# alberthild/vainplex-openclaw

Measured on NVIDIA B200. Metric: messages_scanned_per_s, higher is better.
Workload: dtype u8

## Files before the change

vainplex_openclaw_b200/csrc/bitprog.h:

```cpp
#pragma once
#include <cstdint>
#include "kernels.h"
#include "pike_vm.h"

namespace cg {

constexpr uint32_t kBitProgNone = 0xffffffffu;
constexpr uint32_t kBitCtxs = 32;
CG_HD uint32_t bitprog_meta_off(uint32_t W) { return (128u + kBitCtxs) * W; }
CG_HD uint32_t bitprog_rows_off(uint32_t W) { return bitprog_meta_off(W) + 7u + 2u * W; }
CG_HD uint32_t bitprog_words(uint32_t W, uint32_t n_rows) { return bitprog_rows_off(W) + n_rows * 64u * W * W; }

CG_HD uint32_t bitprog_ctx(int prev, int next, bool at_start) {
  return (uint32_t)(is_word(prev) != is_word(next)) | (at_start ? 2u : 0u) | (next < 0 ? 4u : 0u);
}
CG_HD uint32_t bitprog_in128(uint64_t lo, uint64_t hi, int u) { return u < 0 || u >= 0x80 ? 0u : (uint32_t)(((u & 64) ? hi : lo) >> (u & 63)) & 1u; }

template <int W>
CG_HD int bitprog_test_w(const uint64_t* __restrict__ bp, const uint8_t* __restrict__ m, uint32_t len, uint32_t s, uint32_t t0, uint32_t max_steps, const uint64_t* __restrict__ resume = nullptr) {
  const uint64_t* accept = bp; const uint64_t* start = bp + 128 * W; const uint64_t* hd = bp + bitprog_meta_off(W); const uint64_t* rows = bp + bitprog_rows_off(W);
  const uint64_t meta = hd[0], map0 = hd[1], map1 = hd[2];
  const bool start_same = (meta >> 8) & 1u, has_look = (meta >> 9) & 1u, one_row = (meta & 15u) == 1u;
  const uint64_t lb0 = has_look ? hd[3] : 0, lb1 = has_look ? hd[4] : 0, la0 = has_look ? hd[5] : 0, la1 = has_look ? hd[6] : 0;
  uint64_t m_next[W], m_self[W], live[W], acc_cur[W], start0[W];
  constexpr uint64_t kMatch = 1ull << 63;
  for (int w = 0; w < W; w++) { m_next[w] = hd[7 + w]; m_self[w] = hd[7 + W + w]; }
  int prev = s > 0 ? (m[s - 1] < 0x80 ? (int)m[s - 1] : 0x80) : -1;
  int cur = s < len ? (int)m[s] : -1;
  uint32_t ctx = bitprog_ctx(prev, cur, s == 0) | (has_look ? bitprog_in128(lb0, lb1, prev) << 3 | bitprog_in128(la0, la1, cur) << 4 : 0u);
  for (int w = 0; w < W; w++) { start0[w] = resume ? 0 : start[ctx * W + w]; live[w] = resume ? resume[w] : start0[w]; acc_cur[w] = cur >= 0 && cur < 0x80 ? accept[cur * W + w] : 0; }
  if (resume) t0 = s - 1;
  for (uint32_t pos = s;;) {
    int nb[4]; uint64_t na[4][W];
#ifdef __CUDA_ARCH__
#pragma unroll
#endif
    for (int i = 0; i < 4; i++) nb[i] = pos + 1 + i < len ? (int)m[pos + 1 + i] : -1;
#ifdef __CUDA_ARCH__
#pragma unroll
#endif
    for (int i = 0; i < 4; i++) for (int w = 0; w < W; w++) na[i][w] = nb[i] >= 0 && nb[i] < 0x80 ? accept[nb[i] * W + w] : 0;
#ifdef __CUDA_ARCH__
#pragma unroll
#endif
    for (int i = 0; i < 4; i++) {
      if (live[W - 1] & kMatch) return 1;
      if (cur < 0) return 0;
      if (cur >= 0x80 || pos - s >= max_steps) return -1;
      const int nxt = nb[i];
      uint64_t hit[W], carry = 0, any_hit = 0;
      for (int w = 0; w < W; w++) {
        const uint64_t h = live[w] & acc_cur[w], hn = h & m_next[w];
        live[w] = (hn << 1) | carry | (h & m_self[w]);
        carry = hn >> 63;
        hit[w] = h & ~(m_next[w] | m_self[w]); any_hit |= hit[w];
      }
      if (!start_same || any_hit) ctx = bitprog_ctx(cur, nxt < 0x80 ? nxt : 0x80, false) | (has_look ? bitprog_in128(lb0, lb1, cur) << 3 | bitprog_in128(la0, la1, nxt) << 4 : 0u);
      if (any_hit) {
        const uint32_t row = one_row ? 0u : (uint32_t)(((ctx & 16u) ? map1 : map0) >> (4 * (ctx & 15u))) & 15u;
        const uint64_t* fw = rows + (size_t)row * 64 * W * W;
        for (int w = 0; w < W; w++) {
          uint64_t hw = hit[w];
          while (hw) {
#if defined(__CUDA_ARCH__)
            const int k = __ffsll((long long)hw) - 1;
#else
            const int k = __builtin_ctzll(hw);
#endif
            hw &= hw - 1;
            for (int v = 0; v < W; v++) live[v] |= fw[(size_t)(w * 64 + k) * W + v];
          }
        }
      }
      pos++;
      if (pos <= t0) { for (int w = 0; w < W; w++) live[w] |= start_same ? start0[w] : start[ctx * W + w]; }
      else { uint64_t any = 0; for (int w = 0; w < W; w++) any |= live[w]; if (!any) return 0; }
      cur = nxt;
      for (int w = 0; w < W; w++) acc_cur[w] = na[i][w];
    }
  }
}
CG_HD int bitprog_test(const uint64_t* __restrict__ bp, const uint8_t* __restrict__ m, uint32_t len, uint32_t s, uint32_t t0, uint32_t max_steps = 0xffffffffu, const uint64_t* __restrict__ resume = nullptr) {
  return bp[0] == 2 ? bitprog_test_w<2>(bp + 1, m, len, s, t0, max_steps, resume) : bitprog_test_w<1>(bp + 1, m, len, s, t0, max_steps, resume);
}

CG_HD uint32_t bitprog_sel8(const uint32_t a[8], uint32_t i) {
  const uint32_t lo = (i & 2u) ? ((i & 1u) ? a[3] : a[2]) : ((i & 1u) ? a[1] : a[0]);
  const uint32_t hi = (i & 2u) ? ((i & 1u) ? a[7] : a[6]) : ((i & 1u) ? a[5] : a[4]);
  return (i & 4u) ? hi : lo;
}

CG_HD uint32_t island_start(const DevRuleset& rs, uint32_t rule, const uint8_t* __restrict__ m, uint32_t len, uint32_t t0, uint32_t pre_units, uint32_t limit = 0xffffffffu) {
  const uint32_t pa = pre_units >> 16; pre_units &= 0xffffu;
  const uint32_t* alpha = pa != 0xffffu ? rs.bytesets + (size_t)pa * 8 : rs.rule_alpha + (size_t)rule * 8;
  if (t0 > len) t0 = len;
  uint32_t s = t0;
  uint32_t floor_ = pre_units < 0xffffu ? (t0 > 3u * pre_units ? t0 - 3u * pre_units : 0u) : 0u;
  if (limit != 0xffffffffu && t0 - floor_ > limit) floor_ = t0 - limit - (t0 > limit ? 1u : 0u);
  if (s <= floor_) return s;
  uint32_t a[8];
#ifdef __CUDA_ARCH__
#pragma unroll
#endif
  for (int i = 0; i < 8; i++) a[i] = alpha[i];
  for (;;) {
    uint32_t b[4];
#ifdef __CUDA_ARCH__
#pragma unroll
#endif
    for (uint32_t i = 0; i < 4; i++) b[i] = s > floor_ + i ? m[s - 1 - i] : 0x100u;
#ifdef __CUDA_ARCH__
#pragma unroll
#endif
    for (uint32_t i = 0; i < 4; i++) {
      if (b[i] > 0xffu || !((bitprog_sel8(a, b[i] >> 5) >> (b[i] & 31u)) & 1u)) return s;
      s--;
    }
  }
}


CG_HD int island_test(const DevRuleset& rs, uint32_t f, uint32_t r, const uint8_t* __restrict__ m, uint32_t len, uint32_t t0, uint32_t pre, uint32_t max_steps) {
  const uint64_t* bp = reinterpret_cast<const uint64_t*>(rs.bit_words) + rs.bit_off[r];
  const uint64_t* resume = nullptr; uint32_t s = 0;
  if (f != 0xffffffffu && rs.factor_skip) {
    const uint64_t* sk = reinterpret_cast<const uint64_t*>(rs.factor_skip) + (size_t)f * 3;
    const uint32_t L = (uint32_t)sk[0];
    if (L && t0 + L <= len) { resume = sk + 1; s = t0 + L; }
  }
  if (!resume) {
    s = island_start(rs, r, m, len, t0, pre, max_steps);
    if (max_steps != 0xffffffffu && (t0 < len ? t0 : len) - s >= max_steps) return -1;
  }
  return bitprog_test(bp, m, len, s, t0, max_steps, resume);
}

}
```

vainplex_openclaw_b200/csrc/capi.cu:

```cuda
#include <cuda_runtime.h>

#include <algorithm>
#include <cstdio>
#include <cstdlib>
#include <cstring>
#include <memory>
#include <dlfcn.h>
#include <mutex>
#include <string>
#include <vector>

#include "../../include/openclaw_gov.h"
#include "kernels.h"
#include "rulec.h"
#include "ruleset_image.h"

using namespace cg;

namespace {

thread_local std::string g_err;
std::mutex g_mu;

struct Ctx {
// ... 58 lines not shown
  std::vector<void*> allocs;
  uint32_t n_sets = 0, program_words = 0;
  ScanWork work{};
  uint64_t seq = 0;
  static constexpr int kMirror = 16;
  uint32_t* h_counters = nullptr; cudaEvent_t e_cnt[kMirror] = {}; bool cnt_pending[kMirror] = {};
  uint32_t grow_l1 = 0, grow_slot = 0, grow_ev = 0;
  uint32_t sticky_flags = 0;
  int verify_ctas = 1;
  void size_verify_grid() { const uint32_t ev = last_counters[1]; if (ev > 2048u) verify_ctas = 4; else if (ev < 256u) verify_ctas = 1; }
  uint32_t last_counters[kCounterWords] = {};
  struct CachedGraph { int kernels = 0; cudaGraphExec_t exec = nullptr; const void* bytes = nullptr; const void* off = nullptr; void* words = nullptr; uint32_t n = 0; uint64_t caps[4] = {0, 0, 0, 0}; uint64_t used = 0; };
  struct OnePath { cudaGraphExec_t exec = nullptr; uint8_t* h_pin = nullptr; uint8_t* d_buf = nullptr; uint64_t caps[4] = {0, 0, 0, 0}; int kernels = 0; } one;
  CachedGraph graphs[2];
  uint64_t graph_clock = 0;
  ~cg_ruleset() {
    for (auto& g : graphs) if (g.exec) cudaGraphExecDestroy(g.exec);
    if (one.exec) cudaGraphExecDestroy(one.exec);
    if (one.h_pin) cudaFreeHost(one.h_pin);
    cudaFree(one.d_buf);
    if (h_counters) cudaFreeHost(h_counters);
    for (auto& e : e_cnt) if (e) cudaEventDestroy(e);
    for (void* p : allocs) cudaFree(p);
    cudaFree(work.heavy_idx); cudaFree(work.l1_pos); cudaFree(work.l1_fac); cudaFree(work.fq); cudaFree(work.slot_of_msg);
    cudaFree(work.counters); cudaFree(work.persist); cudaFree(work.slot_msg); cudaFree(work.cand); cudaFree(work.hit); cudaFree(work.events); cudaFree(work.event_pos); cudaFree(work.event_pre); cudaFree(work.spans);
  }
};

namespace {

template <typename T>
int upload(cg_ruleset* rs, const std::vector<T>& v, const T** out, size_t pad_elems = 4) {
  void* d = nullptr;
  size_t bytes = (v.size() + pad_elems) * sizeof(T);
  CU(cudaMalloc(&d, bytes));
  rs->allocs.push_back(d);
  CU(cudaMemset(d, 0, bytes));
  if (!v.empty()) CU(cudaMemcpy(d, v.data(), v.size() * sizeof(T), cudaMemcpyHostToDevice));
  *out = reinterpret_cast<const T*>(d);
  return CG_OK;
}

int ensure_work(cg_ruleset* rs, ScanWork& w, uint32_t n_msgs, uint32_t l1_cap, uint32_t slot_cap, uint32_t event_cap, uint32_t span_cap) {
  if (!w.counters) { CU(cudaMalloc((void**)&w.counters, kCounterWords * sizeof(uint32_t))); CU(cudaMalloc((void**)&w.persist, 16)); CU(cudaMemset(w.persist, 0, 16)); CU(cudaDeviceSynchronize()); }
  if (n_msgs > w.msg_cap) { cudaFree(w.slot_of_msg); w.slot_of_msg = nullptr; w.msg_cap = 0; CU(cudaMalloc((void**)&w.slot_of_msg, (size_t)n_msgs * 4)); w.msg_cap = n_msgs; }
  if (l1_cap > w.l1_cap) {
    cudaFree(w.l1_pos); cudaFree(w.l1_fac); cudaFree(w.fq); w.l1_pos = w.l1_fac = nullptr; w.fq = nullptr; w.l1_cap = 0;
    CU(cudaMalloc((void**)&w.l1_pos, (size_t)l1_cap * 4)); CU(cudaMalloc((void**)&w.l1_fac, (size_t)l1_cap * 4)); CU(cudaMalloc((void**)&w.fq, (size_t)l1_cap * 8));
    w.l1_cap = l1_cap;
  }
  if (slot_cap > w.slot_cap) {
    cudaFree(w.slot_msg); cudaFree(w.cand); cudaFree(w.hit); w.slot_msg = w.cand = w.hit = nullptr; w.slot_cap = 0;
    size_t rw = rs->dev.rw ? rs->dev.rw : 1;
    CU(cudaMalloc((void**)&w.slot_msg, (size_t)slot_cap * 4));
    CU(cudaMalloc((void**)&w.cand, (size_t)slot_cap * rw * 4));
    CU(cudaMalloc((void**)&w.hit, (size_t)slot_cap * rw * 4));
    CU(cudaMemset(w.cand, 0, (size_t)slot_cap * rw * 4)); CU(cudaMemset(w.hit, 0, (size_t)slot_cap * rw * 4)); CU(cudaMemset(w.persist, 0, 16)); CU(cudaDeviceSynchronize());
    w.slot_cap = slot_cap;
  }
  if (event_cap > w.event_cap) { cudaFree(w.events); cudaFree(w.event_pos); cudaFree(w.event_pre); cudaFree(w.heavy_idx); w.events = nullptr; w.event_pos = w.event_pre = w.heavy_idx = nullptr; w.event_cap = 0; CU(cudaMalloc((void**)&w.events, (size_t)event_cap * sizeof(uint2))); CU(cudaMalloc((void**)&w.heavy_idx, (size_t)event_cap * 4)); CU(cudaMalloc((void**)&w.event_pos, (size_t)event_cap * 4)); CU(cudaMalloc((void**)&w.event_pre, (size_t)event_cap * 4)); w.event_cap = event_cap; }
  if (span_cap > w.span_cap) { cudaFree(w.spans); w.spans = nullptr; w.span_cap = 0; CU(cudaMalloc((void**)&w.spans, (size_t)span_cap * 24)); w.span_cap = span_cap; }
  return CG_OK;
}

static uint32_t scan_pieces() { static const uint32_t k = [] { const char* e = getenv("CG_PIECES"); const int v = e ? atoi(e) : 1; return (uint32_t)(v >= 1 && v <= 4 ? v : 1); }(); return k; }
int run_scan_device(cg_ruleset* rs, const uint8_t* d_bytes, const uint32_t* d_off, uint32_t n, uint64_t* d_words, bool spans, cudaStream_t st) {
  const ScanWork& w = rs->work;
  int k = launch_reset(rs->dev, w, n, G.sm_count, st);
  if (G.profiling) cudaEventRecord(G.pev[0], st);
  const uint32_t K = scan_pieces();
  if (G.profiling) G.prof_pieces = K;
// ... 1212 lines not shown
```

vainplex_openclaw_b200/csrc/kernels.h:

```cpp
#pragma once
#include <cuda_runtime.h>
#include <cstdint>

namespace cg {

struct DevRuleset {
  const uint8_t* image;
  uint32_t image_bytes;
  uint32_t stride;
  uint32_t bm_mask, bloom2;
  uint32_t rk_off, rk_mask;
  uint32_t tables_resident;
  uint32_t dir_off, ent_off;
  uint32_t nb_shift;
  uint32_t n_shapes, shapes[16];
  uint32_t n_trig, trig_byte[2];
  uint32_t hot_c5f, hot_c10, hot_one;
  const uint32_t* trig_offsets;
  const uint32_t* trig_list;
  const uint32_t* bucket_start;
  const uint2* entries;
  const uint4* slots;
  const uint32_t* group_entries;
  uint32_t slot_shift, slot_mask;
// ... 2 lines not shown
  uint32_t max_prog_len;
  uint32_t debug_flags;
  const uint32_t* factors;
  const uint32_t* bytesets;
  const uint32_t* always_rules;
  uint32_t n_always;
  const uint32_t* prog;
  const uint32_t* rule_prog_off;
  const uint32_t* sets;
  const uint16_t* set_ranges;
  const unsigned long long* bit_words; const uint32_t* bit_off;
  const unsigned long long* factor_skip;
  const uint32_t* rule_first;
  const uint32_t* rule_alpha;
  const uint32_t* rule_policy; const uint32_t* rule_action;
  uint32_t n_rules;
  uint32_t rw;
};

struct ScanWork {
  uint32_t* counters;
  uint32_t* l1_pos;
  uint32_t* l1_fac;
  uint2* fq;
  uint32_t* persist;
  uint32_t* slot_of_msg;
  uint32_t* slot_msg;
  uint32_t* cand;
  uint32_t* hit;
  uint2* events;
  uint32_t* heavy_idx;
  uint32_t* event_pos;
  uint32_t* event_pre;
  uint32_t* spans;
  uint32_t l1_cap, msg_cap, slot_cap, event_cap, span_cap;
  uint32_t q_cap, q_slot;
};

enum : uint32_t { ERR_EVENT_OVERFLOW = 1, ERR_SPAN_OVERFLOW = 2, ERR_VM_STACK = 4, ERR_VM_LIST = 8, ERR_SLOT_OVERFLOW = 16, ERR_L1_OVERFLOW = 32 };
constexpr uint32_t kCounterWords = 32;
constexpr uint32_t kConfirmTableBudget = 176u * 1024u;
constexpr uint64_t kWordIncomplete = ~0ull;

int launch_scan(const DevRuleset& rs, const ScanWork& w, const uint8_t* d_bytes, const uint32_t* d_off, uint32_t n,
                uint64_t* d_words, int sm_count, cudaStream_t stream);
int launch_confirm(const DevRuleset& rs, const ScanWork& w, const uint8_t* d_bytes, const uint32_t* d_off, uint32_t n, int sm_count, cudaStream_t stream);
int launch_resolve(const DevRuleset& rs, const ScanWork& w, const uint8_t* d_bytes, const uint32_t* d_off, uint32_t n, bool want_spans, int sm_count, cudaStream_t stream);
int launch_verify(const DevRuleset& rs, const ScanWork& w, const uint8_t* d_bytes, const uint32_t* d_off,
                  bool want_spans, int sm_count, cudaStream_t stream, int ctas_per_sm = 4);
int launch_verdicts(const DevRuleset& rs, const ScanWork& w, uint32_t* d_verdicts, int sm_count, cudaStream_t stream);
int launch_finalize(const DevRuleset& rs, const ScanWork& w, uint64_t* d_words, uint32_t n, int sm_count, cudaStream_t stream);
int launch_reset(const DevRuleset& rs, const ScanWork& w, uint32_t n, int sm_count, cudaStream_t stream);

int launch_pack_one(const DevRuleset& rs, const ScanWork& w, const uint64_t* d_word, uint32_t* d_out, uint32_t rw_cap, cudaStream_t stream);

void prepare_scan_kernels();

int launch_sha256_batch(const uint8_t* d_bytes, const uint64_t* d_off, uint32_t n, uint8_t* d_out, cudaStream_t stream);
int launch_merkle_chain(const uint32_t* d_left, uint32_t n_left, const uint32_t* d_acc_in, uint32_t* d_acc_out, cudaStream_t stream);
int launch_merkle_verify(const uint32_t* d_leaf32, uint64_t index, uint64_t size, const uint32_t* d_path, uint32_t path_len, const uint32_t* d_root32, uint32_t* d_ok, cudaStream_t stream);
int launch_redact_digests(const uint8_t* d_bytes, const uint32_t* d_start, const uint32_t* d_len, uint32_t ns, uint32_t* d_out, cudaStream_t stream);
int launch_redact_splice(const uint8_t* d_bytes, const uint32_t* d_off, const uint32_t* d_out_off, const uint32_t* d_span_begin,
                         const uint32_t* d_span_start, const uint32_t* d_span_len, const uint32_t* d_span_cat, const uint32_t* d_digests,
// ... 11 lines not shown
```

vainplex_openclaw_b200/csrc/scan_kernels.cu:

```cuda
#include "kernels.h"
#include "rulec.h"
#include "pike_vm.h"
#include "bitprog.h"
#include "gram_filter.h"
#include <algorithm>

namespace cg {

__device__ __forceinline__ uint32_t smem_u32(const void* p) { return (uint32_t)__cvta_generic_to_shared(p); }
__device__ __forceinline__ void mbar_init(uint64_t* bar, uint32_t count) {
  asm volatile("mbarrier.init.shared::cta.b64 [%0], %1;" ::"r"(smem_u32(bar)), "r"(count));
}
__device__ __forceinline__ void fence_barrier_init() { asm volatile("fence.mbarrier_init.release.cluster;" ::: "memory"); }
__device__ __forceinline__ void fence_proxy_async() { asm volatile("fence.proxy.async.shared::cta;" ::: "memory"); }
__device__ __forceinline__ void mbar_expect_tx(uint64_t* bar, uint32_t bytes) {
  asm volatile("mbarrier.arrive.expect_tx.shared::cta.b64 _, [%0], %1;" ::"r"(smem_u32(bar)), "r"(bytes) : "memory");
}
__device__ __forceinline__ void tma_bulk_g2s(void* dst, const void* src, uint32_t bytes, uint64_t* bar) {
  asm volatile("cp.async.bulk.shared::cluster.global.mbarrier::complete_tx::bytes [%0], [%1], %2, [%3];"
               ::"r"(smem_u32(dst)), "l"(src), "r"(bytes), "r"(smem_u32(bar)) : "memory");
}
__device__ __forceinline__ void mbar_wait(uint64_t* bar, uint32_t phase) {
  asm volatile(
      "{\n"
// ... 179 lines not shown
    h1 += k;
  };
#pragma unroll 1
  while (c - lane < end_chunk) {
    scan_tile(bA, tA, bB, tB, c);
    scan_tile(bB, tB, bA, tA, c + cstep);
    scan_tile(bA, tA, bB, tB, c + 2u * cstep);
    scan_tile(bB, tB, bA, tA, c + 3u * cstep);
    c += 4u * cstep;
    const uint32_t m = __ballot_sync(FULL, acc != 0);
    if (m) {
      if (acc) asm volatile("st.shared.v2.u32 [%0], {%1, %2};" ::"r"(ring1 + (((t1 + __popc(m & lt)) & (kRing - 1)) << 3)), "r"(c), "r"(acc) : "memory");
      t1 += __popc(m); acc = 0;
      if (t1 - h1 >= 32u) { __syncwarp(); append32(32u); }
    }
  }
  __syncwarp();
  if (t1 != h1) append32(t1 - h1);
}

constexpr uint32_t kIslandSteps = 96;
struct SlotSink {
  const DevRuleset& rs; const ScanWork& w; uint32_t msg; uint32_t slot;
  const uint8_t* text = nullptr; uint32_t text_len = 0;
  __device__ SlotSink(const DevRuleset& r, const ScanWork& wk, uint32_t m, bool ws) : rs(r), w(wk), msg(m), slot(0xffffffffu), want_spans(ws) {}
  __device__ bool ensure_slot() {
    if (slot != 0xffffffffu) return slot < w.slot_cap;
    uint32_t s = *reinterpret_cast<volatile uint32_t*>(&w.slot_of_msg[msg]);
    if (s == 0xffffffffu) {
      uint32_t mine = atomicAdd(&w.counters[0], 1u);
      if (mine >= w.slot_cap) { atomicOr(&w.counters[3], ERR_SLOT_OVERFLOW); slot = mine; return false; }
      w.slot_msg[mine] = msg;
      uint32_t old = atomicCAS(&w.slot_of_msg[msg], 0xffffffffu, mine);
      if (old == 0xffffffffu) s = mine; else { s = old; w.slot_msg[mine] = 0xffffffffu; }
    }
    slot = s;
    return true;
  }
  bool want_spans;
  __device__ void candidate(uint32_t r, uint32_t t0, uint32_t pre, uint32_t f) {
    if (!want_spans && text && rs.bit_words) {
      const uint32_t bo = rs.bit_off[r];
      if (bo != kBitProgNone) {
        if (slot == 0xffffffffu) { const uint32_t s0 = *reinterpret_cast<volatile uint32_t*>(&w.slot_of_msg[msg]); if (s0 != 0xffffffffu && s0 < w.slot_cap && ((w.hit[(size_t)s0 * rs.rw + (r >> 5)] >> (r & 31)) & 1u)) return; }
        const int res = island_test(rs, f, r, text, text_len, t0, pre, kIslandSteps);
        if (res == 0) return;
        if (res == 1) { direct(r); return; }
      }
    }
    if (!ensure_slot()) return;
    uint32_t bit = 1u << (r & 31);
    uint32_t old = atomicOr(&w.cand[(size_t)slot * rs.rw + (r >> 5)], bit);
    if (want_spans && (old & bit)) return;
    uint32_t e = atomicAdd(&w.counters[1], 1u);
    if (e < w.event_cap) {
      const bool heavy = !want_spans && (pre & 0xffffu) >= 24u;
      w.events[e] = make_uint2(slot, r | (heavy ? 0x80000000u : 0u)); w.event_pos[e] = t0; w.event_pre[e] = pre;
      if (heavy) w.heavy_idx[atomicAdd(&w.counters[17], 1u)] = e;
    } else atomicOr(&w.counters[3], ERR_EVENT_OVERFLOW);
  }
  __device__ void candidate_always(uint32_t r) {
    if (!ensure_slot()) return;
    uint32_t bit = 1u << (r & 31);
    uint32_t old = atomicOr(&w.cand[(size_t)slot * rs.rw + (r >> 5)], bit);
    if (old & bit) return;
    uint32_t e = atomicAdd(&w.counters[1], 1u);
    if (e < w.event_cap) { w.events[e] = make_uint2(slot, r); w.event_pos[e] = 0xffffffffu; } else atomicOr(&w.counters[3], ERR_EVENT_OVERFLOW);
  }
  __device__ void direct(uint32_t r) {
    if (!ensure_slot()) return;
    uint32_t bit = 1u << (r & 31);
    atomicOr(&w.cand[(size_t)slot * rs.rw + (r >> 5)], bit);
// ... 128 lines not shown
  uint32_t head = 0, tail = 0, flagged = 0;
  for (uint32_t base = gwarp * 32u; base < nq; base += nwarps * 32u) {
    uint2 q = make_uint2(0u, 0u);
    if (base + lane < nq) q = w.fq[base + lane];
    uint32_t bits = q.y;
    for (;;) {
      const uint32_t m = __ballot_sync(FULL, bits != 0);
      if (!m) break;
      if (bits) {
        const uint32_t bit = (uint32_t)__ffs((int)bits) - 1u; bits &= bits - 1u;
        ring[(tail + __popc(m & lt)) & (kCfRing - 1)] = ((q.x - (bit / kbits + 1u) * cstep) * kbits + (kbits - 1u - bit % kbits)) << kshift;
      }
      tail += __popc(m); flagged += lane == 0 ? __popc(m) : 0u;
      __syncwarp();
      if (tail - head >= 32u) { const uint32_t pos = ring[(head + lane) & (kCfRing - 1)]; head += 32u; __syncwarp(); confirm_gram(c, pos, true); }
    }
  }
  if (tail != head) { const bool a = lane < tail - head; const uint32_t pos = a ? ring[(head + lane) & (kCfRing - 1)] : 0u; __syncwarp(); confirm_gram(c, pos, a); }
  if (c.ptail != c.phead) { const bool a = lane < c.ptail - c.phead; const uint2 pr = a ? c.pring[(c.phead + lane) & (kCfRing - 1)] : make_uint2(0u, 0u); confirm_pairs(c, pr, a); }
  const uint32_t passed = __reduce_add_sync(FULL, c.passed);
  if (lane == 0) { if (flagged) atomicAdd(&w.counters[6], flagged); if (passed) atomicAdd(&w.counters[19], passed); if (c.ptail) atomicAdd(&w.counters[28 + w.q_slot], c.ptail); }
}

__global__ void __launch_bounds__(256, 4)
resolve_kernel(DevRuleset rs, ScanWork w, const uint8_t* __restrict__ bytes, const uint32_t* __restrict__ off, uint32_t n, int want_spans, uint32_t spread) {
  const uint32_t n1 = min(w.counters[4], w.l1_cap);
  const uint32_t stride = gridDim.x * blockDim.x, tid = blockIdx.x * blockDim.x + threadIdx.x;
  for (uint32_t i = tid / spread; i < n1 && tid % spread == 0; i += stride / spread) {
    const uint32_t pos = w.l1_pos[i], f = w.l1_fac[i];
    const uint32_t msg = message_of(off, n, pos);
    if (pos + (rs.factors[(size_t)f * 12 + 1] & 0xffu) > off[msg + 1]) continue;
    SlotSink sink(rs, w, msg, want_spans != 0);
    sink.text = bytes + off[msg]; sink.text_len = off[msg + 1] - off[msg];
    factor_confirmed(rs, f, pos - off[msg], want_spans != 0, sink);
  }
  if (rs.n_always) for (uint32_t msg = tid; msg < n; msg += stride) {
    SlotSink sink(rs, w, msg, want_spans != 0);
    for (uint32_t k = 0; k < rs.n_always; k++) sink.candidate_always(rs.always_rules[k]);
  }
}

constexpr int kVerifyThreads = 64;
constexpr int kVerifyBlock = 256, kVerifyCtasPerSm = 4, kVerifySlots = kVerifyBlock / 32;
constexpr int kSmallProg = 192;

struct GlobalSpanSink {
  const ScanWork& w; uint32_t msg, rule; bool lane0_only;
  __device__ void span(uint32_t sb, uint32_t eb, uint32_t s16, uint32_t e16) {
    if (lane0_only && (threadIdx.x & 31u)) return;
    uint32_t k = atomicAdd(&w.counters[2], 1u);
    if (k < w.span_cap) { uint32_t* o = w.spans + (size_t)k * 6; o[0] = msg; o[1] = rule; o[2] = sb; o[3] = eb; o[4] = s16; o[5] = e16; }
    else atomicOr(&w.counters[3], ERR_SPAN_OVERFLOW);
  }
};

struct SmemStore {
  static constexpr uint32_t cap = kSmallProg;
  static constexpr bool coop = true;
  uint16_t* mark_; uint16_t* pcs_; uint32_t* sts_; uint16_t* stk_; uint32_t stride, t;
  __device__ __forceinline__ uint16_t& mark(uint32_t i) { return mark_[i * stride + t]; }
  __device__ __forceinline__ uint16_t& pc(int L, uint32_t i) { return pcs_[(L * cap + i) * stride + t]; }
// ... 115 lines not shown

__global__ void verdict_kernel(DevRuleset rs, ScanWork w, uint32_t* __restrict__ verdicts) {
  const uint32_t n_slots = min(w.counters[0], w.slot_cap);
  for (uint32_t s = blockIdx.x * blockDim.x + threadIdx.x; s < n_slots; s += gridDim.x * blockDim.x) {
    const uint32_t msg = w.slot_msg[s];
    if (msg == 0xffffffffu) continue;
    uint32_t prev = 0xffffffffu, best = 0, decide = 0xfffffu, matched = 0;
    for (uint32_t k = 0; k < rs.rw; k++) {
      uint32_t v = w.hit[(size_t)s * rs.rw + k];
      while (v) {
        const uint32_t r = k * 32 + (__ffs(v) - 1); v &= v - 1;
        const uint32_t p = rs.rule_policy[r];
        if (p == prev) continue;
        prev = p; matched++;
        const uint32_t a = rs.rule_action[r];
        if (a == 2u && best != 2u) { best = 2u; decide = r; } else if (a == 1u && best == 0u) { best = 1u; decide = r; }
      }
    }
    if (matched) verdicts[msg] = best | (min(matched, 1023u) << 2) | (decide << 12);
  }
}

#define CG_FOR_SCAN_VARIANTS(X) X(1, 0, 0) X(1, 1, 0) X(1, 2, 0) X(2, 0, 0) X(2, 1, 0) X(2, 2, 0) X(1, 0, 1) X(1, 1, 1) X(1, 2, 1) X(2, 0, 1) X(2, 1, 1) X(2, 2, 1)
static int scan_threads() { static int t = 0; if (!t) { t = kScanThreads; if (const char* e = getenv("CG_SCAN_THREADS")) { int v = atoi(e); if (v == 512 || v == 768 || v == 1024) t = v; } } return t; }
void prepare_scan_kernels() {
  int dev = 0, optin = 0; cudaGetDevice(&dev); cudaDeviceGetAttribute(&optin, cudaDevAttrMaxSharedMemoryPerBlockOptin, dev);
  const int kMaxSmem = (optin > 0 ? optin : 227 * 1024) - 1024;
#define CG_PREP(P, T, B) cudaFuncSetAttribute(scan_kernel<P, T, B, 1024>, cudaFuncAttributeMaxDynamicSharedMemorySize, kMaxSmem); \
  cudaFuncSetAttribute(scan_kernel<P, T, B, 768>, cudaFuncAttributeMaxDynamicSharedMemorySize, kMaxSmem); cudaFuncSetAttribute(scan_kernel<P, T, B, 512>, cudaFuncAttributeMaxDynamicSharedMemorySize, kMaxSmem);
  CG_FOR_SCAN_VARIANTS(CG_PREP)
#undef CG_PREP
  cudaFuncSetAttribute(confirm_kernel, cudaFuncAttributeMaxDynamicSharedMemorySize, (int)(kCfRingBytes + kConfirmTableBudget));
  cudaFuncSetAttribute(verify_small_kernel<true>, cudaFuncAttributeMaxDynamicSharedMemorySize, (int)kVerifySmem);
  cudaFuncSetAttribute(verify_small_kernel<false>, cudaFuncAttributeMaxDynamicSharedMemorySize, (int)kVerifySmem);
}

static uint32_t scan_grid(uint32_t n, int sm_count) {
  uint32_t grid = (uint32_t)sm_count;
  if (n < 4096) grid = std::max<uint32_t>(1u, std::min<uint32_t>(grid, n / 32u + 1u));
  return grid;
}
int launch_scan(const DevRuleset& rs, const ScanWork& w, const uint8_t* d_bytes, const uint32_t* d_off, uint32_t n,
                uint64_t* d_words, int sm_count, cudaStream_t stream) {
  if (n == 0) return 0;
  const size_t smem = (size_t)rs.image_bytes + kScanRingBytes;
  const uint32_t grid = scan_grid(n, sm_count);
  const int np = rs.stride == 2 ? 2 : 1, nt = (int)rs.n_trig, bl = rs.bloom2 ? 1 : 0, th = scan_threads();
#define CG_LAUNCH(P, T, B) if (np == P && nt == T && bl == B) { \
    if (th == 1024) scan_kernel<P, T, B, 1024><<<grid, 1024, smem, stream>>>(rs, w, d_bytes, d_off, n, d_words); \
    else if (th == 768) scan_kernel<P, T, B, 768><<<grid, 768, smem, stream>>>(rs, w, d_bytes, d_off, n, d_words); \
    else scan_kernel<P, T, B, 512><<<grid, 512, smem, stream>>>(rs, w, d_bytes, d_off, n, d_words); }
  CG_FOR_SCAN_VARIANTS(CG_LAUNCH)
#undef CG_LAUNCH
  return 1;
}

int launch_confirm(const DevRuleset& rs, const ScanWork& w, const uint8_t* d_bytes, const uint32_t* d_off, uint32_t n, int sm_count, cudaStream_t stream) {
  if (n == 0) return 0;
  const uint32_t cstep = scan_grid(n, sm_count) * (uint32_t)(scan_threads() / 32) * 32u;
  confirm_kernel<<<scan_grid(n, sm_count), kCfThreads, (size_t)kCfRingBytes + (rs.cf_resident ? rs.cf_bytes : 0u), stream>>>(rs, w, d_bytes, d_off, n, cstep);
  return 1;
}
int launch_resolve(const DevRuleset& rs, const ScanWork& w, const uint8_t* d_bytes, const uint32_t* d_off, uint32_t n, bool want_spans, int sm_count, cudaStream_t stream) {
  if (n == 0) return 0;
  static const uint32_t spread = [] { const char* e = getenv("CG_RESOLVE_SPREAD"); const int v = e ? atoi(e) : 4; return (uint32_t)(v == 1 || v == 2 || v == 4 || v == 8 || v == 16 || v == 32 ? v : 4); }();
  resolve_kernel<<<sm_count * 8, 256, 0, stream>>>(rs, w, d_bytes, d_off, n, want_spans ? 1 : 0, spread);
  return 1;
}

int launch_verify(const DevRuleset& rs, const ScanWork& w, const uint8_t* d_bytes, const uint32_t* d_off,
                  bool want_spans, int sm_count, cudaStream_t stream, int ctas_per_sm) {
  int k = 1;
  static const int forced = [] { const char* e = getenv("CG_VERIFY_CTAS"); const int v = e ? atoi(e) : 0; return v >= 1 && v <= kVerifyCtasPerSm ? v : 0; }();
  const int ctas = forced ? forced : (ctas_per_sm >= 1 && ctas_per_sm <= kVerifyCtasPerSm ? ctas_per_sm : kVerifyCtasPerSm);
  if (want_spans) {
    verify_small_kernel<true><<<sm_count * ctas, kVerifyBlock, kVerifySmem, stream>>>(rs, w, d_bytes, d_off);
  } else {
    verify_small_kernel<false><<<sm_count * ctas, kVerifyBlock, kVerifySmem, stream>>>(rs, w, d_bytes, d_off);
  }
  if (rs.max_prog_len > (uint32_t)kSmallProg) {
    k++;
    if (want_spans) verify_large_kernel<true><<<sm_count * 4, kVerifyThreads, 0, stream>>>(rs, w, d_bytes, d_off);
    else verify_large_kernel<false><<<sm_count * 4, kVerifyThreads, 0, stream>>>(rs, w, d_bytes, d_off);
  }
  return k;
}

int launch_verdicts(const DevRuleset& rs, const ScanWork& w, uint32_t* d_verdicts, int sm_count, cudaStream_t stream) {
  verdict_kernel<<<sm_count * 2, 256, 0, stream>>>(rs, w, d_verdicts);
  return 1;
// ... 26 lines not shown
```

Before: 5.122 billion.

## Split resolve into classify and persistent warp-refilled island-walk queue kernels

The resolve stage no longer runs island bit-program walks inline, one thread per level-1 hit. It now classifies hits into per-width queues, and a second kernel drains those queues with warps that refill idle lanes from an atomic cursor. The walk runs incrementally in blocks of four bytes through a resumable state struct. The goal is to remove lane divergence from walks of very different lengths and to separate the width-1 and width-2 programs. The cost is an extra kernel launch, a global queue buffer, and atomics on counter slots that must be reset between batches.

```diff
diff --git a/vainplex_openclaw_b200/csrc/bitprog.h b/vainplex_openclaw_b200/csrc/bitprog.h
--- a/vainplex_openclaw_b200/csrc/bitprog.h
+++ b/vainplex_openclaw_b200/csrc/bitprog.h
@@ -16,123 +16,147 @@
 }
 CG_HD uint32_t bitprog_in128(uint64_t lo, uint64_t hi, int u) { return u < 0 || u >= 0x80 ? 0u : (uint32_t)(((u & 64) ? hi : lo) >> (u & 63)) & 1u; }
 
+constexpr int kWalkMore = 2;
 template <int W>
-CG_HD int bitprog_test_w(const uint64_t* __restrict__ bp, const uint8_t* __restrict__ m, uint32_t len, uint32_t s, uint32_t t0, uint32_t max_steps, const uint64_t* __restrict__ resume = nullptr) {
-  const uint64_t* accept = bp; const uint64_t* start = bp + 128 * W; const uint64_t* hd = bp + bitprog_meta_off(W); const uint64_t* rows = bp + bitprog_rows_off(W);
-  const uint64_t meta = hd[0], map0 = hd[1], map1 = hd[2];
-  const bool start_same = (meta >> 8) & 1u, has_look = (meta >> 9) & 1u, one_row = (meta & 15u) == 1u;
-  const uint64_t lb0 = has_look ? hd[3] : 0, lb1 = has_look ? hd[4] : 0, la0 = has_look ? hd[5] : 0, la1 = has_look ? hd[6] : 0;
-  uint64_t m_next[W], m_self[W], live[W], acc_cur[W], start0[W];
-  constexpr uint64_t kMatch = 1ull << 63;
-  for (int w = 0; w < W; w++) { m_next[w] = hd[7 + w]; m_self[w] = hd[7 + W + w]; }
-  int prev = s > 0 ? (m[s - 1] < 0x80 ? (int)m[s - 1] : 0x80) : -1;
-  int cur = s < len ? (int)m[s] : -1;
-  uint32_t ctx = bitprog_ctx(prev, cur, s == 0) | (has_look ? bitprog_in128(lb0, lb1, prev) << 3 | bitprog_in128(la0, la1, cur) << 4 : 0u);
-  for (int w = 0; w < W; w++) { start0[w] = resume ? 0 : start[ctx * W + w]; live[w] = resume ? resume[w] : start0[w]; acc_cur[w] = cur >= 0 && cur < 0x80 ? accept[cur * W + w] : 0; }
-  if (resume) t0 = s - 1;
-  for (uint32_t pos = s;;) {
-    int nb[4]; uint64_t na[4][W];
-#ifdef __CUDA_ARCH__
-#pragma unroll
-#endif
-    for (int i = 0; i < 4; i++) nb[i] = pos + 1 + i < len ? (int)m[pos + 1 + i] : -1;
-#ifdef __CUDA_ARCH__
-#pragma unroll
-#endif
-    for (int i = 0; i < 4; i++) for (int w = 0; w < W; w++) na[i][w] = nb[i] >= 0 && nb[i] < 0x80 ? accept[nb[i] * W + w] : 0;
-#ifdef __CUDA_ARCH__
-#pragma unroll
-#endif
-    for (int i = 0; i < 4; i++) {
-      if (live[W - 1] & kMatch) return 1;
-      if (cur < 0) return 0;
-      if (cur >= 0x80 || pos - s >= max_steps) return -1;
-      const int nxt = nb[i];
-      uint64_t hit[W], carry = 0, any_hit = 0;
-      for (int w = 0; w < W; w++) {
-        const uint64_t h = live[w] & acc_cur[w], hn = h & m_next[w];
-        live[w] = (hn << 1) | carry | (h & m_self[w]);
-        carry = hn >> 63;
-        hit[w] = h & ~(m_next[w] | m_self[w]); any_hit |= hit[w];
-      }
-      if (!start_same || any_hit) ctx = bitprog_ctx(cur, nxt < 0x80 ? nxt : 0x80, false) | (has_look ? bitprog_in128(lb0, lb1, cur) << 3 | bitprog_in128(la0, la1, nxt) << 4 : 0u);
-      if (any_hit) {
-        const uint32_t row = one_row ? 0u : (uint32_t)(((ctx & 16u) ? map1 : map0) >> (4 * (ctx & 15u))) & 15u;
-        const uint64_t* fw = rows + (size_t)row * 64 * W * W;
-        for (int w = 0; w < W; w++) {
-          uint64_t hw = hit[w];
-          while (hw) {
-#if defined(__CUDA_ARCH__)
-            const int k = __ffsll((long long)hw) - 1;
-#else
-            const int k = __builtin_ctzll(hw);
-#endif
-            hw &= hw - 1;
-            for (int v = 0; v < W; v++) live[v] |= fw[(size_t)(w * 64 + k) * W + v];
-          }
-        }
-      }
-      pos++;
-      if (pos <= t0) { for (int w = 0; w < W; w++) live[w] |= start_same ? start0[w] : start[ctx * W + w]; }
-      else { uint64_t any = 0; for (int w = 0; w < W; w++) any |= live[w]; if (!any) return 0; }
-      cur = nxt;
-      for (int w = 0; w < W; w++) acc_cur[w] = na[i][w];
-    }
+struct IslandWalk {
+  const uint64_t* bp;
+  uint64_t m_next[W], m_self[W], start0[W], map0, map1, lb0, lb1, la0, la1;
+  bool start_same, has_look, one_row, seek;
+  const uint8_t* m; uint32_t len, t0, s;
+  const uint32_t* alpha; uint32_t floor_;
+  uint64_t live[W], acc_cur[W];
+  uint32_t pos, ctx; int cur;
+};
+
+template <int W>
+CG_HD void island_walk_begin(IslandWalk<W>& st, const uint64_t* __restrict__ resume) {
+  const uint64_t* accept = st.bp; const uint64_t* start = st.bp + 128 * W;
+  const uint32_t s = st.s;
+  const int prev = s > 0 ? (st.m[s - 1] < 0x80 ? (int)st.m[s - 1] : 0x80) : -1;
+  const int cur = s < st.len ? (int)st.m[s] : -1;
+  st.ctx = bitprog_ctx(prev, cur, s == 0) | (st.has_look ? bitprog_in128(st.lb0, st.lb1, prev) << 3 | bitprog_in128(st.la0, st.la1, cur) << 4 : 0u);
+  for (int w = 0; w < W; w++) {
+    st.start0[w] = resume ? 0 : start[st.ctx * W + w];
+    st.live[w] = resume ? resume[w] : st.start0[w];
+    st.acc_cur[w] = cur >= 0 && cur < 0x80 ? accept[cur * W + w] : 0;
   }
-}
-CG_HD int bitprog_test(const uint64_t* __restrict__ bp, const uint8_t* __restrict__ m, uint32_t len, uint32_t s, uint32_t t0, uint32_t max_steps = 0xffffffffu, const uint64_t* __restrict__ resume = nullptr) {
-  return bp[0] == 2 ? bitprog_test_w<2>(bp + 1, m, len, s, t0, max_steps, resume) : bitprog_test_w<1>(bp + 1, m, len, s, t0, max_steps, resume);
+  if (resume) st.t0 = s - 1;
+  st.pos = s; st.cur = cur; st.seek = false;
 }
 
-CG_HD uint32_t bitprog_sel8(const uint32_t a[8], uint32_t i) {
-  const uint32_t lo = (i & 2u) ? ((i & 1u) ? a[3] : a[2]) : ((i & 1u) ? a[1] : a[0]);
-  const uint32_t hi = (i & 2u) ? ((i & 1u) ? a[7] : a[6]) : ((i & 1u) ? a[5] : a[4]);
-  return (i & 4u) ? hi : lo;
+template <int W>
+CG_HD void island_walk_init(IslandWalk<W>& st, const DevRuleset& rs, uint32_t r, const uint8_t* __restrict__ m, uint32_t len, uint32_t t0,
+                            uint32_t pre, const uint64_t* __restrict__ skip, uint32_t max_steps) {
+  st.bp = reinterpret_cast<const uint64_t*>(rs.bit_words) + rs.bit_off[r] + 1;
+  const uint64_t* hd = st.bp + bitprog_meta_off(W);
+  const uint64_t meta = hd[0];
+  st.map0 = hd[1]; st.map1 = hd[2];
+  st.start_same = (meta >> 8) & 1u; st.has_look = (meta >> 9) & 1u; st.one_row = (meta & 15u) == 1u;
+  st.lb0 = st.has_look ? hd[3] : 0; st.lb1 = st.has_look ? hd[4] : 0; st.la0 = st.has_look ? hd[5] : 0; st.la1 = st.has_look ? hd[6] : 0;
+  for (int w = 0; w < W; w++) { st.m_next[w] = hd[7 + w]; st.m_self[w] = hd[7 + W + w]; }
+  st.m = m; st.len = len; st.t0 = t0;
+  if (skip) { st.s = t0 + (uint32_t)skip[0]; island_walk_begin(st, skip + 1); return; }
+  const uint32_t pa = pre >> 16, pu = pre & 0xffffu;
+  st.alpha = pa != 0xffffu ? rs.bytesets + (size_t)pa * 8 : rs.rule_alpha + (size_t)r * 8;
+  const uint32_t tc = t0 < len ? t0 : len;
+  st.s = tc;
+  st.floor_ = pu < 0xffffu ? (tc > 3u * pu ? tc - 3u * pu : 0u) : 0u;
+  if (max_steps != 0xffffffffu && tc - st.floor_ > max_steps) st.floor_ = tc - max_steps - (tc > max_steps ? 1u : 0u);
+  st.seek = true;
 }
 
-CG_HD uint32_t island_start(const DevRuleset& rs, uint32_t rule, const uint8_t* __restrict__ m, uint32_t len, uint32_t t0, uint32_t pre_units, uint32_t limit = 0xffffffffu) {
-  const uint32_t pa = pre_units >> 16; pre_units &= 0xffffu;
-  const uint32_t* alpha = pa != 0xffffu ? rs.bytesets + (size_t)pa * 8 : rs.rule_alpha + (size_t)rule * 8;
-  if (t0 > len) t0 = len;
-  uint32_t s = t0;
-  uint32_t floor_ = pre_units < 0xffffu ? (t0 > 3u * pre_units ? t0 - 3u * pre_units : 0u) : 0u;
-  if (limit != 0xffffffffu && t0 - floor_ > limit) floor_ = t0 - limit - (t0 > limit ? 1u : 0u);
-  if (s <= floor_) return s;
-  uint32_t a[8];
-#ifdef __CUDA_ARCH__
-#pragma unroll
-#endif
-  for (int i = 0; i < 8; i++) a[i] = alpha[i];
-  for (;;) {
+template <int W>
+CG_HD int island_walk_block(IslandWalk<W>& st, uint32_t max_steps) {
+  if (st.seek) {
     uint32_t b[4];
 #ifdef __CUDA_ARCH__
 #pragma unroll
 #endif
-    for (uint32_t i = 0; i < 4; i++) b[i] = s > floor_ + i ? m[s - 1 - i] : 0x100u;
+    for (uint32_t i = 0; i < 4; i++) b[i] = st.s > st.floor_ + i ? st.m[st.s - 1 - i] : 0x100u;
+    bool found = false;
 #ifdef __CUDA_ARCH__
 #pragma unroll
 #endif
     for (uint32_t i = 0; i < 4; i++) {
-      if (b[i] > 0xffu || !((bitprog_sel8(a, b[i] >> 5) >> (b[i] & 31u)) & 1u)) return s;
-      s--;
+      if (!found && (b[i] > 0xffu || !((st.alpha[b[i] >> 5] >> (b[i] & 31u)) & 1u))) found = true;
+      if (!found) st.s--;
     }
+    if (!found) return kWalkMore;
+    if (max_steps != 0xffffffffu && (st.t0 < st.len ? st.t0 : st.len) - st.s >= max_steps) return -1;
+    island_walk_begin(st, nullptr);
+    return kWalkMore;
   }
+  const uint64_t* accept = st.bp; const uint64_t* start = st.bp + 128 * W; const uint64_t* rows = st.bp + bitprog_rows_off(W);
+  constexpr uint64_t kMatch = 1ull << 63;
+  int nb[4]; uint64_t na[4][W];
+#ifdef __CUDA_ARCH__
+#pragma unroll
+#endif
+  for (int i = 0; i < 4; i++) nb[i] = st.pos + 1 + i < st.len ? (int)st.m[st.pos + 1 + i] : -1;
+#ifdef __CUDA_ARCH__
+#pragma unroll
+#endif
+  for (int i = 0; i < 4; i++) for (int w = 0; w < W; w++) na[i][w] = nb[i] >= 0 && nb[i] < 0x80 ? accept[nb[i] * W + w] : 0;
+#ifdef __CUDA_ARCH__
+#pragma unroll
+#endif
+  for (int i = 0; i < 4; i++) {
+    if (st.live[W - 1] & kMatch) return 1;
+    if (st.cur < 0) return 0;
+    if (st.cur >= 0x80 || st.pos - st.s >= max_steps) return -1;
+    const int nxt = nb[i];
+    uint64_t hit[W], carry = 0, any_hit = 0;
+    for (int w = 0; w < W; w++) {
+      const uint64_t h = st.live[w] & st.acc_cur[w], hn = h & st.m_next[w];
+      st.live[w] = (hn << 1) | carry | (h & st.m_self[w]);
+      carry = hn >> 63;
+      hit[w] = h & ~(st.m_next[w] | st.m_self[w]); any_hit |= hit[w];
+    }
+    if (!st.start_same || any_hit) st.ctx = bitprog_ctx(st.cur, nxt < 0x80 ? nxt : 0x80, false) | (st.has_look ? bitprog_in128(st.lb0, st.lb1, st.cur) << 3 | bitprog_in128(st.la0, st.la1, nxt) << 4 : 0u);
+    if (any_hit) {
+      const uint32_t row = st.one_row ? 0u : (uint32_t)(((st.ctx & 16u) ? st.map1 : st.map0) >> (4 * (st.ctx & 15u))) & 15u;
+      const uint64_t* fw = rows + (size_t)row * 64 * W * W;
+      for (int w = 0; w < W; w++) {
+        uint64_t hw = hit[w];
+        while (hw) {
+#if defined(__CUDA_ARCH__)
+          const int k = __ffsll((long long)hw) - 1;
+#else
+          const int k = __builtin_ctzll(hw);
+#endif
+          hw &= hw - 1;
+          for (int v = 0; v < W; v++) st.live[v] |= fw[(size_t)(w * 64 + k) * W + v];
+        }
+      }
+    }
+    st.pos++;
+    if (st.pos <= st.t0) { for (int w = 0; w < W; w++) st.live[w] |= st.start_same ? st.start0[w] : start[st.ctx * W + w]; }
+    else { uint64_t any = 0; for (int w = 0; w < W; w++) any |= st.live[w]; if (!any) return 0; }
+    st.cur = nxt;
+    for (int w = 0; w < W; w++) st.acc_cur[w] = na[i][w];
+  }
+  return kWalkMore;
 }
 
+CG_HD const uint64_t* island_skip(const DevRuleset& rs, uint32_t f, uint32_t len, uint32_t t0) {
+  if (f == 0xffffffffu || !rs.factor_skip) return nullptr;
+  const uint64_t* sk = reinterpret_cast<const uint64_t*>(rs.factor_skip) + (size_t)f * 3;
+  const uint32_t L = (uint32_t)sk[0];
+  return L && t0 + L <= len ? sk : nullptr;
+}
+CG_HD uint32_t bitprog_width(const DevRuleset& rs, uint32_t r) { return (uint32_t)(reinterpret_cast<const uint64_t*>(rs.bit_words)[rs.bit_off[r]]); }
 
+template <int W>
+CG_HD int island_test_w(const DevRuleset& rs, uint32_t r, const uint8_t* __restrict__ m, uint32_t len, uint32_t t0, uint32_t pre, const uint64_t* skip, uint32_t max_steps) {
+  IslandWalk<W> st;
+  island_walk_init(st, rs, r, m, len, t0, pre, skip, max_steps);
+  int res;
+  while ((res = island_walk_block(st, max_steps)) == kWalkMore) {}
+  return res;
+}
 CG_HD int island_test(const DevRuleset& rs, uint32_t f, uint32_t r, const uint8_t* __restrict__ m, uint32_t len, uint32_t t0, uint32_t pre, uint32_t max_steps) {
-  const uint64_t* bp = reinterpret_cast<const uint64_t*>(rs.bit_words) + rs.bit_off[r];
-  const uint64_t* resume = nullptr; uint32_t s = 0;
-  if (f != 0xffffffffu && rs.factor_skip) {
-    const uint64_t* sk = reinterpret_cast<const uint64_t*>(rs.factor_skip) + (size_t)f * 3;
-    const uint32_t L = (uint32_t)sk[0];
-    if (L && t0 + L <= len) { resume = sk + 1; s = t0 + L; }
-  }
-  if (!resume) {
-    s = island_start(rs, r, m, len, t0, pre, max_steps);
-    if (max_steps != 0xffffffffu && (t0 < len ? t0 : len) - s >= max_steps) return -1;
-  }
-  return bitprog_test(bp, m, len, s, t0, max_steps, resume);
+  const uint64_t* skip = island_skip(rs, f, len, t0);
+  return bitprog_width(rs, r) == 2 ? island_test_w<2>(rs, r, m, len, t0, pre, skip, max_steps) : island_test_w<1>(rs, r, m, len, t0, pre, skip, max_steps);
 }
 
 }
diff --git a/vainplex_openclaw_b200/csrc/capi.cu b/vainplex_openclaw_b200/csrc/capi.cu
--- a/vainplex_openclaw_b200/csrc/capi.cu
+++ b/vainplex_openclaw_b200/csrc/capi.cu
@@ -104,7 +104,7 @@
     if (h_counters) cudaFreeHost(h_counters);
     for (auto& e : e_cnt) if (e) cudaEventDestroy(e);
     for (void* p : allocs) cudaFree(p);
-    cudaFree(work.heavy_idx); cudaFree(work.l1_pos); cudaFree(work.l1_fac); cudaFree(work.fq); cudaFree(work.slot_of_msg);
+    cudaFree(work.heavy_idx); cudaFree(work.l1_pos); cudaFree(work.l1_fac); cudaFree(work.fq); cudaFree(work.walk); cudaFree(work.slot_of_msg);
     cudaFree(work.counters); cudaFree(work.persist); cudaFree(work.slot_msg); cudaFree(work.cand); cudaFree(work.hit); cudaFree(work.events); cudaFree(work.event_pos); cudaFree(work.event_pre); cudaFree(work.spans);
   }
 };
@@ -127,8 +127,9 @@
   if (!w.counters) { CU(cudaMalloc((void**)&w.counters, kCounterWords * sizeof(uint32_t))); CU(cudaMalloc((void**)&w.persist, 16)); CU(cudaMemset(w.persist, 0, 16)); CU(cudaDeviceSynchronize()); }
   if (n_msgs > w.msg_cap) { cudaFree(w.slot_of_msg); w.slot_of_msg = nullptr; w.msg_cap = 0; CU(cudaMalloc((void**)&w.slot_of_msg, (size_t)n_msgs * 4)); w.msg_cap = n_msgs; }
   if (l1_cap > w.l1_cap) {
-    cudaFree(w.l1_pos); cudaFree(w.l1_fac); cudaFree(w.fq); w.l1_pos = w.l1_fac = nullptr; w.fq = nullptr; w.l1_cap = 0;
+    cudaFree(w.l1_pos); cudaFree(w.l1_fac); cudaFree(w.fq); cudaFree(w.walk); w.l1_pos = w.l1_fac = nullptr; w.fq = nullptr; w.walk = nullptr; w.l1_cap = 0;
     CU(cudaMalloc((void**)&w.l1_pos, (size_t)l1_cap * 4)); CU(cudaMalloc((void**)&w.l1_fac, (size_t)l1_cap * 4)); CU(cudaMalloc((void**)&w.fq, (size_t)l1_cap * 8));
+    CU(cudaMalloc((void**)&w.walk, (size_t)l1_cap * sizeof(uint4)));
     w.l1_cap = l1_cap;
   }
   if (slot_cap > w.slot_cap) {
diff --git a/vainplex_openclaw_b200/csrc/kernels.h b/vainplex_openclaw_b200/csrc/kernels.h
--- a/vainplex_openclaw_b200/csrc/kernels.h
+++ b/vainplex_openclaw_b200/csrc/kernels.h
@@ -48,6 +48,7 @@
   uint32_t* counters;
   uint32_t* l1_pos;
   uint32_t* l1_fac;
+  uint4* walk;
   uint2* fq;
   uint32_t* persist;
   uint32_t* slot_of_msg;
@@ -65,6 +66,8 @@
 
 enum : uint32_t { ERR_EVENT_OVERFLOW = 1, ERR_SPAN_OVERFLOW = 2, ERR_VM_STACK = 4, ERR_VM_LIST = 8, ERR_SLOT_OVERFLOW = 16, ERR_L1_OVERFLOW = 32 };
 constexpr uint32_t kCounterWords = 32;
+constexpr uint32_t kCtrWalkQueued = 20;
+constexpr uint32_t kCtrWalkCursor = 22;
 constexpr uint32_t kConfirmTableBudget = 176u * 1024u;
 constexpr uint64_t kWordIncomplete = ~0ull;
 
diff --git a/vainplex_openclaw_b200/csrc/scan_kernels.cu b/vainplex_openclaw_b200/csrc/scan_kernels.cu
--- a/vainplex_openclaw_b200/csrc/scan_kernels.cu
+++ b/vainplex_openclaw_b200/csrc/scan_kernels.cu
@@ -225,7 +225,6 @@
 constexpr uint32_t kIslandSteps = 96;
 struct SlotSink {
   const DevRuleset& rs; const ScanWork& w; uint32_t msg; uint32_t slot;
-  const uint8_t* text = nullptr; uint32_t text_len = 0;
   __device__ SlotSink(const DevRuleset& r, const ScanWork& wk, uint32_t m, bool ws) : rs(r), w(wk), msg(m), slot(0xffffffffu), want_spans(ws) {}
   __device__ bool ensure_slot() {
     if (slot != 0xffffffffu) return slot < w.slot_cap;
@@ -240,17 +239,12 @@
     slot = s;
     return true;
   }
+  __device__ bool known_hit(uint32_t r) const {
+    const uint32_t s0 = *reinterpret_cast<volatile uint32_t*>(&w.slot_of_msg[msg]);
+    return s0 != 0xffffffffu && s0 < w.slot_cap && ((w.hit[(size_t)s0 * rs.rw + (r >> 5)] >> (r & 31)) & 1u);
+  }
   bool want_spans;
-  __device__ void candidate(uint32_t r, uint32_t t0, uint32_t pre, uint32_t f) {
-    if (!want_spans && text && rs.bit_words) {
-      const uint32_t bo = rs.bit_off[r];
-      if (bo != kBitProgNone) {
-        if (slot == 0xffffffffu) { const uint32_t s0 = *reinterpret_cast<volatile uint32_t*>(&w.slot_of_msg[msg]); if (s0 != 0xffffffffu && s0 < w.slot_cap && ((w.hit[(size_t)s0 * rs.rw + (r >> 5)] >> (r & 31)) & 1u)) return; }
-        const int res = island_test(rs, f, r, text, text_len, t0, pre, kIslandSteps);
-        if (res == 0) return;
-        if (res == 1) { direct(r); return; }
-      }
-    }
+  __device__ void candidate(uint32_t r, uint32_t t0, uint32_t pre) {
     if (!ensure_slot()) return;
     uint32_t bit = 1u << (r & 31);
     uint32_t old = atomicOr(&w.cand[(size_t)slot * rs.rw + (r >> 5)], bit);
@@ -425,21 +419,104 @@
   if (lane == 0) { if (flagged) atomicAdd(&w.counters[6], flagged); if (passed) atomicAdd(&w.counters[19], passed); if (c.ptail) atomicAdd(&w.counters[28 + w.q_slot], c.ptail); }
 }
 
-__global__ void __launch_bounds__(256, 4)
-resolve_kernel(DevRuleset rs, ScanWork w, const uint8_t* __restrict__ bytes, const uint32_t* __restrict__ off, uint32_t n, int want_spans, uint32_t spread) {
+struct ClassifySink {
+  SlotSink slots; uint32_t len;
+  uint32_t q = 0; uint4 d = make_uint4(0, 0, 0, 0);
+  __device__ ClassifySink(const DevRuleset& r, const ScanWork& wk, uint32_t m, uint32_t l, bool ws) : slots(r, wk, m, ws), len(l) {}
+  __device__ void direct(uint32_t r) { slots.direct(r); }
+  __device__ void candidate(uint32_t r, uint32_t t0, uint32_t pre, uint32_t f) {
+    const DevRuleset& rs = slots.rs;
+    if (slots.want_spans || !rs.bit_words || rs.bit_off[r] == kBitProgNone) { slots.candidate(r, t0, pre); return; }
+    q = bitprog_width(rs, r);
+    d = make_uint4(slots.msg, r | (island_skip(rs, f, len, t0) ? 0x80000000u : 0u), t0, f);
+  }
+};
+
+__global__ void __launch_bounds__(256)
+resolve_classify_kernel(DevRuleset rs, ScanWork w, const uint32_t* __restrict__ off, uint32_t n, int want_spans) {
   const uint32_t n1 = min(w.counters[4], w.l1_cap);
   const uint32_t stride = gridDim.x * blockDim.x, tid = blockIdx.x * blockDim.x + threadIdx.x;
-  for (uint32_t i = tid / spread; i < n1 && tid % spread == 0; i += stride / spread) {
-    const uint32_t pos = w.l1_pos[i], f = w.l1_fac[i];
-    const uint32_t msg = message_of(off, n, pos);
-    if (pos + (rs.factors[(size_t)f * 12 + 1] & 0xffu) > off[msg + 1]) continue;
-    SlotSink sink(rs, w, msg, want_spans != 0);
-    sink.text = bytes + off[msg]; sink.text_len = off[msg + 1] - off[msg];
-    factor_confirmed(rs, f, pos - off[msg], want_spans != 0, sink);
+  const uint32_t lane = threadIdx.x & 31u, lt = (1u << lane) - 1u, FULL = 0xffffffffu;
+  for (uint32_t i = tid; i - lane < n1; i += stride) {
+    uint32_t q = 0; uint4 d;
+    if (i < n1) {
+      const uint32_t pos = w.l1_pos[i], f = w.l1_fac[i];
+      const uint32_t msg = message_of(off, n, pos);
+      if (pos + (rs.factors[(size_t)f * 12 + 1] & 0xffu) <= off[msg + 1]) {
+        ClassifySink sink(rs, w, msg, off[msg + 1] - off[msg], want_spans != 0);
+        factor_confirmed(rs, f, pos - off[msg], want_spans != 0, sink);
+        q = sink.q; d = sink.d;
+      }
+    }
+#pragma unroll
+    for (uint32_t k = 1; k <= 2; k++) {
+      const uint32_t m = __ballot_sync(FULL, q == k);
+      if (!m) continue;
+      const uint32_t leader = __ffs((int)m) - 1u;
+      uint32_t base = 0;
+      if (lane == leader) base = atomicAdd(&w.counters[kCtrWalkQueued + k - 1], __popc(m));
+      base = __shfl_sync(FULL, base, leader) + __popc(m & lt);
+      if (q == k) w.walk[k == 1 ? base : w.l1_cap - 1u - base] = d;
+    }
   }
   if (rs.n_always) for (uint32_t msg = tid; msg < n; msg += stride) {
     SlotSink sink(rs, w, msg, want_spans != 0);
     for (uint32_t k = 0; k < rs.n_always; k++) sink.candidate_always(rs.always_rules[k]);
+  }
+}
+
+template <int W>
+__device__ __forceinline__ void walk_queue(const DevRuleset& rs, const ScanWork& w, const uint8_t* __restrict__ bytes, const uint32_t* __restrict__ off, uint32_t lanes) {
+  const uint32_t lane = threadIdx.x & 31u, lt = (1u << lane) - 1u, FULL = 0xffffffffu;
+  const uint32_t nq = w.counters[kCtrWalkQueued + W - 1];
+  uint32_t* cursor = &w.counters[kCtrWalkCursor + W - 1];
+  IslandWalk<W> st;
+  uint4 d = make_uint4(0, 0, 0, 0);
+  bool busy = false, more = true;
+  for (;;) {
+    const uint32_t idle = __ballot_sync(FULL, !busy) & lanes;
+    if (more && idle) {
+      uint32_t base = 0;
+      if (lane == 0) base = atomicAdd(cursor, __popc(idle));
+      base = __shfl_sync(FULL, base, 0);
+      more = base + __popc(idle) < nq;
+      const uint32_t j = base + __popc(idle & lt);
+      if (((idle >> lane) & 1u) && j < nq) {
+        d = w.walk[W == 1 ? j : w.l1_cap - 1u - j];
+        const uint32_t r = d.y & 0x7fffffffu;
+        busy = !SlotSink(rs, w, d.x, false).known_hit(r);
+        if (busy) {
+          const uint32_t mb = off[d.x], len = off[d.x + 1] - mb;
+          const uint32_t* fw = rs.factors + (size_t)d.w * 12;
+          island_walk_init(st, rs, r, bytes + mb, len, d.z, fw[10] | (fw[11] << 16),
+                           (d.y >> 31) ? reinterpret_cast<const uint64_t*>(rs.factor_skip) + (size_t)d.w * 3 : nullptr, kIslandSteps);
+        }
+      }
+    }
+    if (!__any_sync(FULL, busy)) { if (more) continue; break; }
+    if (busy) {
+      const int res = island_walk_block(st, kIslandSteps);
+      if (res != kWalkMore) {
+        busy = false;
+        const uint32_t r = d.y & 0x7fffffffu;
+        SlotSink sink(rs, w, d.x, false);
+        if (res == 1) sink.direct(r);
+        else if (res < 0) { const uint32_t* fw = rs.factors + (size_t)d.w * 12; sink.candidate(r, d.z, fw[10] | (fw[11] << 16)); }
+      }
+    }
+  }
+}
+
+__global__ void __launch_bounds__(256, 2)
+resolve_walk_kernel(DevRuleset rs, ScanWork w, const uint8_t* __restrict__ bytes, const uint32_t* __restrict__ off) {
+  const uint32_t n1 = w.counters[kCtrWalkQueued], n2 = w.counters[kCtrWalkQueued + 1];
+  const uint32_t nw = gridDim.x * (blockDim.x >> 5), g = (threadIdx.x >> 5) * gridDim.x + blockIdx.x;
+  const bool one_first = g < (n1 + n2 ? (uint32_t)(((uint64_t)nw * n1 + (n1 + n2) / 2) / (n1 + n2)) : nw);
+  const uint32_t per_warp = min(32u, max(1u, (n1 + n2 + nw - 1) / nw));
+  const uint32_t lanes = per_warp == 32 ? 0xffffffffu : (1u << per_warp) - 1u;
+  for (int pass = 0; pass < 2; pass++) {
+    if (one_first == (pass == 0)) walk_queue<1>(rs, w, bytes, off, lanes);
+    else walk_queue<2>(rs, w, bytes, off, lanes);
   }
 }
 
@@ -601,6 +678,7 @@
 }
 
 #define CG_FOR_SCAN_VARIANTS(X) X(1, 0, 0) X(1, 1, 0) X(1, 2, 0) X(2, 0, 0) X(2, 1, 0) X(2, 2, 0) X(1, 0, 1) X(1, 1, 1) X(1, 2, 1) X(2, 0, 1) X(2, 1, 1) X(2, 2, 1)
+static int g_walk_ctas = 1;
 static int scan_threads() { static int t = 0; if (!t) { t = kScanThreads; if (const char* e = getenv("CG_SCAN_THREADS")) { int v = atoi(e); if (v == 512 || v == 768 || v == 1024) t = v; } } return t; }
 void prepare_scan_kernels() {
   int dev = 0, optin = 0; cudaGetDevice(&dev); cudaDeviceGetAttribute(&optin, cudaDevAttrMaxSharedMemoryPerBlockOptin, dev);
@@ -609,6 +687,7 @@
   cudaFuncSetAttribute(scan_kernel<P, T, B, 768>, cudaFuncAttributeMaxDynamicSharedMemorySize, kMaxSmem); cudaFuncSetAttribute(scan_kernel<P, T, B, 512>, cudaFuncAttributeMaxDynamicSharedMemorySize, kMaxSmem);
   CG_FOR_SCAN_VARIANTS(CG_PREP)
 #undef CG_PREP
+  if (cudaOccupancyMaxActiveBlocksPerMultiprocessor(&g_walk_ctas, resolve_walk_kernel, 256, 0) != cudaSuccess || g_walk_ctas < 1) { cudaGetLastError(); g_walk_ctas = 1; }
   cudaFuncSetAttribute(confirm_kernel, cudaFuncAttributeMaxDynamicSharedMemorySize, (int)(kCfRingBytes + kConfirmTableBudget));
   cudaFuncSetAttribute(verify_small_kernel<true>, cudaFuncAttributeMaxDynamicSharedMemorySize, (int)kVerifySmem);
   cudaFuncSetAttribute(verify_small_kernel<false>, cudaFuncAttributeMaxDynamicSharedMemorySize, (int)kVerifySmem);
@@ -642,9 +721,9 @@
 }
 int launch_resolve(const DevRuleset& rs, const ScanWork& w, const uint8_t* d_bytes, const uint32_t* d_off, uint32_t n, bool want_spans, int sm_count, cudaStream_t stream) {
   if (n == 0) return 0;
-  static const uint32_t spread = [] { const char* e = getenv("CG_RESOLVE_SPREAD"); const int v = e ? atoi(e) : 4; return (uint32_t)(v == 1 || v == 2 || v == 4 || v == 8 || v == 16 || v == 32 ? v : 4); }();
-  resolve_kernel<<<sm_count * 8, 256, 0, stream>>>(rs, w, d_bytes, d_off, n, want_spans ? 1 : 0, spread);
-  return 1;
+  resolve_classify_kernel<<<sm_count * 8, 256, 0, stream>>>(rs, w, d_off, n, want_spans ? 1 : 0);
+  resolve_walk_kernel<<<sm_count * g_walk_ctas, 256, 0, stream>>>(rs, w, d_bytes, d_off);
+  return 2;
 }
 
 int launch_verify(const DevRuleset& rs, const ScanWork& w, const uint8_t* d_bytes, const uint32_t* d_off,
```

Measured after the change: 5.015 billion (median of 6 runs). 0.979x the previous value.
